# martasumyk/hyperspectral_super-resolution

Hardware: AMD Instinct MI355X
Metric: Mpixel*bands/s fused (SRF + deg-3 per-band LSQ fit + apply) (higher is better)
Workload: dtype f32

## Files before the change

hyperspectral_super-resolution_amd/csrc/hsr_srf.hip:

```cpp
#include <hip/hip_ext.h>

#include "hsr_common.h"
#include "hsr_solve.h"
#include "hsr_sync_dev.h"
#include "hsr_fused_dev.h"

namespace hsr {

struct SrfBands {
  int32_t k0[HSR_MAX_BANDS];
  int32_t klen[HSR_MAX_BANDS];
  int32_t woff[HSR_MAX_BANDS];
  int8_t band_of[8][2];
};

constexpr int kWeightCap = 1024;

typedef hsr_batch_unit SrfUnit;
static_assert(sizeof(SrfUnit) == 64 && sizeof(hsr_batch_tile) == 64, "batch records are 64 bytes");

struct SrfFit {
  double* gpart;
  int32_t* tickets;
  double* moments;
  double* coeffs;
  long long min_count;
};

struct SrfArgs {
  SrfFit fit;
  SrfUnit one;
  const SrfUnit* units;
  int32_t nunits;
  int32_t B;
  int32_t ldsB;
  int32_t wtaps;
  const float* wn;
  SrfBands bands;
  int32_t nb;
  int64_t out_bs, out_ps;
  int64_t real_bs, real_ps;
  float min_x, min_y;
  int32_t u16;
  int32_t u16_fast;
  float scale;
  uint32_t nodata;
  const float* apply_x;
  float* apply_out;
  const double* apply_coeffs;
  const uint8_t* apply_mask;
  int64_t apply_npix;
  int32_t apply_clip;
  const double* lazy_partials;
  int32_t lazy_slots;
  long long lazy_min_count;
  double* lazy_moments;
  double* lazy_coeffs;
  unsigned int* lazy_counter;
  unsigned int lazy_base;
  unsigned int* lazy_ready;
  int32_t lazy_group_T;
  int32_t lazy_group_index;
  const double* lazy_group_moments;
  double* lazy_group_total;
  const unsigned int* apply_ready;
  unsigned int apply_ready_value;
  unsigned int* sync_error;
#ifdef HSR_PHASE_STAMPS
  unsigned long long* stamps;
  unsigned long long* stamps2;
  uint32_t* stamps3;
#endif
};

#ifdef HSR_PHASE_STAMPS
unsigned long long* g_stamp_buffer = nullptr;
unsigned long long* g_stamp_buffer2 = nullptr;
uint32_t* g_stamp_buffer3 = nullptr;
__device__ __forceinline__ unsigned long long real_time() {
  unsigned long long t;
  asm volatile("s_memrealtime %0\n\ts_waitcnt lgkmcnt(0)" : "=s"(t)::"memory");
  return t;
}
__device__ __forceinline__ unsigned long long phase_stamp() {
  unsigned long long t;
  asm volatile("s_memtime %0\n\ts_waitcnt lgkmcnt(0)" : "=s"(t)::"memory");
  return t;
}
#define HSR_STAMP(var) const unsigned long long var = phase_stamp()
#else
#define HSR_STAMP(var)
#endif

constexpr int kGroupPixels = 64;
constexpr int kGroups = 8;
constexpr int kBandSlots = HSR_MAX_BANDS / kGroups;
constexpr int kTapChunk = 16;
constexpr int kScanBatch = 5;
constexpr int kScanBatchF32 = 5;

struct SrfTuning {
  int reserved_cus;
  bool u16_ring;
  bool u16_fast;
};

static int srf_tuning(const hsr_srf_options* o, SrfTuning* t, const char* who) {
  t->reserved_cus = 0;
  t->u16_ring = true;
  t->u16_fast = false;
  if (o == nullptr) return HSR_OK;
  HSR_REQUIRE(o->tile_pixels == 0 || o->tile_pixels == 64, HSR_ERR_INVALID,
              "%s: options.tile_pixels must be 0 (default) or 64, got %d (the 32-pixel geometry of round 1 measured 3-8 %% "
              "slower and was removed)", who, o->tile_pixels);
  HSR_REQUIRE(o->reserved_cus >= 0 && o->reserved_cus <= 128, HSR_ERR_INVALID, "%s: options.reserved_cus=%d outside [0,128]",
              who, o->reserved_cus);
  HSR_REQUIRE((o->flags & ~HSR_SRF_U16_FAST) == 0, HSR_ERR_INVALID, "%s: options.flags has unknown bits (0x%x)", who, o->flags);
  t->reserved_cus = o->reserved_cus;
  t->u16_ring = o->u16_single_buffer == 0;
  t->u16_fast = (o->flags & HSR_SRF_U16_FAST) != 0;
  return HSR_OK;
}

static int srf_slots(int64_t npix, int reserved_cus) {
  int64_t groups = (npix + kGroupPixels - 1) / kGroupPixels;
  if (groups < 1) groups = 1;
  const int64_t cap = (int64_t)(256 - reserved_cus) * 2;
  int64_t slots = groups;
  if (groups > 64 && groups <= 512) {
    slots = (groups + 3) / 4;
    if (slots < 64) slots = 64;
  }
  return (int)(slots < cap ? slots : cap);
}

typedef __attribute__((address_space(1))) const void* gptr_t;
typedef __attribute__((address_space(3))) void* lptr_t;

__device__ __forceinline__ void lds_barrier() {
  asm volatile("s_waitcnt lgkmcnt(0)\n\ts_barrier" ::: "memory");
}

__device__ __forceinline__ void stage_f32(const float* p, float* stage_wave_uniform) {
  __builtin_amdgcn_global_load_lds((gptr_t)p, (lptr_t)stage_wave_uniform, 4, 0, 0);
}
__device__ __forceinline__ void stage_u8(const uint8_t* p, uint32_t* stage_wave_uniform) {
  const uintptr_t a = reinterpret_cast<uintptr_t>(p);
  __builtin_amdgcn_global_load_lds((gptr_t)(a & ~(uintptr_t)3), (lptr_t)stage_wave_uniform, 4, 0, 0);
}
__device__ __forceinline__ uint32_t staged_u8(const uint8_t* p, const uint32_t* stage, int lane) {
  return (stage[lane] >> ((reinterpret_cast<uintptr_t>(p) & 3) * 8)) & 0xffu;
}
constexpr int kTargetStageBytesPerBand = 64 * 4;
__host__ __device__ constexpr size_t target_stage_bytes(int nb) { return (size_t)nb * kTargetStageBytesPerBand + 64 * 4; }

__device__ __forceinline__ const char* unit_record_addr(const SrfUnit* units, int64_t idx, int nunits, int lane) {
  const int64_t i = idx < nunits ? idx : (int64_t)nunits - 1;
  return reinterpret_cast<const char*>(units + i) + (lane & 15) * 4;
}
__device__ __forceinline__ SrfUnit unit_from_lds(const uint32_t* us) {
  uint32_t w[15];
#pragma unroll
  for (int i = 0; i < 15; ++i) w[i] = __builtin_amdgcn_readfirstlane(us[i]);
  SrfUnit u;
  u.cube_dev = reinterpret_cast<const void*>(((uint64_t)w[1] << 32) | w[0]);
  u.real_dev = reinterpret_cast<const float*>(((uint64_t)w[3] << 32) | w[2]);
  u.mask_dev = reinterpret_cast<const uint8_t*>(((uint64_t)w[5] << 32) | w[4]);
  u.pseudo_dev = reinterpret_cast<float*>(((uint64_t)w[7] << 32) | w[6]);
  u.part_dev = reinterpret_cast<double*>(((uint64_t)w[9] << 32) | w[8]);
  u.npix = (int64_t)(((uint64_t)w[11] << 32) | w[10]);
  u.slots = (int32_t)w[12];
  u.slot = (int32_t)w[13];
  u.ngroups = (int32_t)w[14];
  u.reserved = 0;
  return u;
}

__device__ __forceinline__ bool any_nonfinite4(const float4& v) {
  float z = v.x * 0.0f;
  z = fmaf(v.y, 0.0f, z);
  z = fmaf(v.z, 0.0f, z);
  z = fmaf(v.w, 0.0f, z);
  return z != z;
}

__host__ __device__ __forceinline__ int stage_row(int nb, int ops) { return ops > nb ? nb : ops; }

template <int T>
__device__ __forceinline__ void flush_stage(const float* ostage, float* out, int64_t pix0, int npx, int nb, int ops, int t) {
  const int n4 = (npx * ops) >> 2;
  float4* dst = reinterpret_cast<float4*>(out + pix0 * ops);
  if (ops == nb) {
    const float4* src = reinterpret_cast<const float4*>(ostage);
    for (int i = t; i < n4; i += T) st_stream(dst + i, src[i]);
    return;
  }
  const int q = ops >> 2;
  for (int i = t; i < n4; i += T) {
    const int px = q == 4 ? i >> 2 : (q == 2 ? i >> 1 : (q == 1 ? i : i / 3));
    const int c = (i - px * q) * 4;
    const float* r = ostage + px * nb + c;
    st_stream(dst + i, make_float4(c < nb ? r[0] : 0.0f, c + 1 < nb ? r[1] : 0.0f, c + 2 < nb ? r[2] : 0.0f, c + 3 < nb ? r[3] : 0.0f));
  }
}

__device__ __forceinline__ double f64_of(int hi, int lo) { return __hiloint2double(hi, lo); }

template <int D>
__device__ __forceinline__ double merge_pair(double a, double b) {
  const int alo = __double2loint(a), ahi = __double2hiint(a), blo = __double2loint(b), bhi = __double2hiint(b);
  if (D == 32) {
    const auto l = __builtin_amdgcn_permlane32_swap(alo, blo, false, false);
    const auto h = __builtin_amdgcn_permlane32_swap(ahi, bhi, false, false);
    return f64_of(h[0], l[0]) + f64_of(h[1], l[1]);
  } else if (D == 16) {
    const auto l = __builtin_amdgcn_permlane16_swap(alo, blo, false, false);
    const auto h = __builtin_amdgcn_permlane16_swap(ahi, bhi, false, false);
    return f64_of(h[0], l[0]) + f64_of(h[1], l[1]);
  } else if (D == 8) {
    const int xlo = __builtin_amdgcn_update_dpp(alo, blo, 0x128, 0xf, 0xC, false), xhi = __builtin_amdgcn_update_dpp(ahi, bhi, 0x128, 0xf, 0xC, false);
    const int ylo = __builtin_amdgcn_update_dpp(blo, alo, 0x128, 0xf, 0x3, false), yhi = __builtin_amdgcn_update_dpp(bhi, ahi, 0x128, 0xf, 0x3, false);
    return f64_of(xhi, xlo) + f64_of(yhi, ylo);
  } else {
    static_assert(D == 32 || D == 16 || D == 8 || D == 4, "merge levels");
    const int xlo = __builtin_amdgcn_update_dpp(alo, blo, 0x124, 0xf, 0xA, false), xhi = __builtin_amdgcn_update_dpp(ahi, bhi, 0x124, 0xf, 0xA, false);
    const int ylo = __builtin_amdgcn_update_dpp(blo, alo, 0x12C, 0xf, 0x5, false), yhi = __builtin_amdgcn_update_dpp(bhi, ahi, 0x12C, 0xf, 0x5, false);
    return f64_of(xhi, xlo) + f64_of(yhi, ylo);
  }
}

template <int D>
__device__ __forceinline__ double plain_level(double v) {
  const int lo = __double2loint(v), hi = __double2hiint(v);
  if (D == 32) {
    const auto l = __builtin_amdgcn_permlane32_swap(lo, lo, false, false);
    const auto h = __builtin_amdgcn_permlane32_swap(hi, hi, false, false);
    return f64_of(h[0], l[0]) + f64_of(h[1], l[1]);
  }
  static_assert(D == 32 || D == 2 || D == 1, "plain levels");
  constexpr int ctrl = D == 2 ? 0x4E : 0xB1;
  return v + f64_of(__builtin_amdgcn_update_dpp(0, hi, ctrl, 0xf, 0xf, false), __builtin_amdgcn_update_dpp(0, lo, ctrl, 0xf, 0xf, false));
}

template <int D, int NIN, int NMAX>
__device__ __forceinline__ void merge_level(double (&v)[NMAX]) {
  constexpr int NOUT = (NIN + 1) / 2;
#pragma unroll
  for (int i = 0; i < NOUT; ++i) v[i] = merge_pair<D>(v[2 * i], v[2 * i + 1 < NIN ? 2 * i + 1 : NIN - 1]);
}

template <int M, int P, bool LANE_IS_PIXEL, bool COHERENT>
__device__ __forceinline__ void flush_moments(double (&acc_m)[2][M], const bool (&bval)[2], const int (&bidx)[2],
                                              double* part, int lane) {
  constexpr int N = 2 * M;
  constexpr bool kTop32 = P == 64 && LANE_IS_PIXEL;
  constexpr int N1 = kTop32 ? (N + 1) / 2 : N, N2 = (N1 + 1) / 2, N3 = (N2 + 1) / 2, N4 = (N3 + 1) / 2;
  double v[N];
#pragma unroll
  for (int j = 0; j < 2; ++j)
#pragma unroll
    for (int m = 0; m < M; ++m) {
      v[j * M + m] = acc_m[j][m];
      acc_m[j][m] = 0.0;
    }
  if (kTop32) merge_level<32, N, N>(v);
  merge_level<16, N1, N>(v);
  merge_level<8, N2, N>(v);
  merge_level<4, N3, N>(v);
#pragma unroll
  for (int q = 0; q < N4; ++q) {
    v[q] = plain_level<1>(plain_level<2>(v[q]));
    if (!LANE_IS_PIXEL) v[q] = plain_level<32>(v[q]);
  }
  const int b2 = (lane >> 2) & 1, b3 = (lane >> 3) & 1, b4 = (lane >> 4) & 1, b5 = (lane >> 5) & 1;
  const bool canonical = (lane & 3) == 0 && (LANE_IS_PIXEL || b5 == 0);
#pragma unroll
  for (int q = 0; q < N4; ++q) {
    int i = 2 * q + b2;
    bool valid = canonical && i < N3;
    i = 2 * i + b3;
    valid = valid && i < N2;
    i = 2 * i + b4;
    valid = valid && i < N1;
    if (kTop32) {
      i = 2 * i + b5;
      valid = valid && i < N;
    }
    const bool second = i >= M;
    if (valid && (second ? bval[1] : bval[0])) {
      double* dst = part + (size_t)(second ? bidx[1] : bidx[0]) * M + (i - (second ? M : 0));
      if (COHERENT)
        __hip_atomic_store(dst, v[q], __ATOMIC_RELAXED, __HIP_MEMORY_SCOPE_AGENT);
      else
        *dst = v[q];
    }
  }
}

template <int DEG>
__device__ __forceinline__ void fused_fit(const SrfFit& f, const double* part, int S, int nb, unsigned char* lds, int t) {
  constexpr int M = moment_count(DEG);
  const int R = nb * M;
  const int grp = (int)blockIdx.x & 63;
  int* flag = reinterpret_cast<int*>(lds);
  double* mom = reinterpret_cast<double*>(lds + 64);
  double* work = mom + HSR_MAX_BANDS * M;
  stores_done_barrier();
  if (t == 0) {
    const int expect = (S - grp + 63) >> 6;
    *flag = __hip_atomic_fetch_add(f.tickets + grp, 1, __ATOMIC_RELAXED, __HIP_MEMORY_SCOPE_AGENT) == expect - 1;
  }
  __syncthreads();
  if (!*flag) return;
  if (t < R) {
    const double* row = part + t;
    double s = 0.0;
    for (int i0 = grp; i0 < S; i0 += 64 * 8) {
      double v[8];
#pragma unroll
      for (int u = 0; u < 8; ++u) {
        const int i = i0 + 64 * u;
        v[u] = i < S ? ld_agent(row + (size_t)i * R) : 0.0;
      }
#pragma unroll
      for (int u = 0; u < 8; ++u) s += v[u];
    }
    st_agent(f.gpart + (size_t)grp * R + t, s);
  }
  stores_done_barrier();
  const int ngroups = S < 64 ? S : 64;
  if (t == 0) *flag = __hip_atomic_fetch_add(f.tickets + 64, 1, __ATOMIC_RELAXED, __HIP_MEMORY_SCOPE_AGENT) == ngroups - 1;
  __syncthreads();
  if (!*flag) return;
  {
    const int lane = t & 63, wave = t >> 6;
    constexpr int RW = (HSR_MAX_BANDS * M + 7) / 8;
    double v[RW];
#pragma unroll
    for (int k = 0; k < RW; ++k) {
      const int r = wave + 8 * k;
      v[k] = (r < R && lane < ngroups) ? ld_agent(f.gpart + (size_t)lane * R + r) : 0.0;
    }
#pragma unroll
    for (int k = 0; k < RW; ++k) {
      const int r = wave + 8 * k;
      const double s = wave_sum(v[k]);
      if (lane == 0 && r < R) {
        mom[r] = s;
        f.moments[r] = s;
      }
    }
  }
  __syncthreads();
  if (t < nb) solve_band_t<DEG, true>(mom + t * M, f.min_count, f.coeffs + (size_t)t * (DEG + 1), work + t * kSolveWork);
  if (t < 65) __hip_atomic_store(f.tickets + t, 0, __ATOMIC_RELAXED, __HIP_MEMORY_SCOPE_AGENT);
}

template <int DEG, bool FAST, bool WLDS, int P, bool OUTV, bool BATCH, bool APPLY = false>
__global__ __launch_bounds__(8 * P, 4) void srf_kernel(const SrfArgs a) {
  constexpr int T = 8 * P;
  constexpr int NW = T / 64;
  extern __shared__ __attribute__((aligned(16))) unsigned char smem[];
  float* tile = reinterpret_cast<float*>(smem);
  const int B = a.B;
  const int ldsB = a.ldsB;
  uint32_t* flags = reinterpret_cast<uint32_t*>(smem + (size_t)P * ldsB * 4);
  uint32_t* ustage = flags + 64;
  const float* wl = reinterpret_cast<const float*>(flags + 64 + (BATCH ? 16 : 0));
  float* ostage = const_cast<float*>(wl) + (WLDS ? a.wtaps : 0);
  const int ops = (int)a.out_ps;
  const int osr = stage_row(a.nb, ops);
  static_assert(P == 64, "one pixel per lane: the target stage is indexed by lane");
  float* ystage = ostage + (OUTV ? P * osr : 0);
  uint32_t* mstage = reinterpret_cast<uint32_t*>(ystage + a.nb * 64);
  float* prev_out = nullptr;
  int64_t prev_pix0 = 0;
  int prev_npx = 0;

#ifdef HSR_PHASE_STAMPS
  const unsigned long long rt_begin = real_time();
#endif
  const int t = threadIdx.x;
  const int lane = t & 63;
  const int wave = __builtin_amdgcn_readfirstlane(t >> 6);
  const int pl = t % P;
  const int grp = wave;
  const int nchunk = P * B / 4;

  if constexpr (APPLY && DEG > 0) apply_prephase<DEG + 1, T>(a, smem, t);

  int bk0[kBandSlots], bkl[kBandSlots], bwo[kBandSlots], bidx[kBandSlots];
  bool bval[kBandSlots];
#pragma unroll
  for (int j = 0; j < kBandSlots; ++j) {
    const int b = a.bands.band_of[grp][j];
    bval[j] = b >= 0;
    bidx[j] = bval[j] ? b : 0;
    const int bb = bidx[j];
    bk0[j] = a.bands.k0[bb];
    bkl[j] = bval[j] ? a.bands.klen[bb] : 0;
    bwo[j] = a.bands.woff[bb];
  }

  bool constants_staged = false;
  auto stage_constants = [&]() {
    if (WLDS) {
      float* wlw = const_cast<float*>(wl);
      for (int b = 0; b < a.nb; ++b) {
        const int kl = a.bands.klen[b];
        for (int i = t; i < kl; i += T) wlw[a.bands.woff[b] + i] = a.wn[(size_t)b * B + a.bands.k0[b] + i];
      }
    }
  };

#ifdef HSR_PHASE_STAMPS
  unsigned long long stamp_acc[8] = {0, 0, 0, 0, 0, 0, 0, 0};
  unsigned long long round_t0 = rt_begin;
  int round_no = 0;
#endif
  constexpr int M = DEG > 0 ? moment_count(DEG) : 1;
  double acc_m[kBandSlots][M];
  if (DEG > 0) {
#pragma unroll
    for (int j = 0; j < kBandSlots; ++j)
#pragma unroll
      for (int m = 0; m < M; ++m) acc_m[j][m] = 0.0;
  }

  SrfUnit cu;
  if (BATCH) {
    cu = a.units[blockIdx.x];
  } else {
    cu = a.one;
    cu.slot = blockIdx.x;
    cu.part_dev = a.one.part_dev + (size_t)blockIdx.x * a.nb * M;
  }
  int64_t nidx = (int64_t)blockIdx.x + gridDim.x;
  int g = cu.slot;
  bool pend = false;
  double* pend_part = nullptr;

  for (bool more = true; more;) {
    const int64_t pix0 = (int64_t)g * P;
    const int64_t left = cu.npix - pix0;
    const int npx = left < P ? (int)left : P;
    const float* src = reinterpret_cast<const float*>(cu.cube_dev) + pix0 * B;
    const bool pvalid = pl < npx;

    float yv[kBandSlots];
    uint32_t mraw = 1u;
    auto load_targets = [&]() {
      if (DEG > 0) {
        const int64_t pc = pvalid ? pix0 + pl : cu.npix - 1;
#pragma unroll
        for (int j = 0; j < kBandSlots; ++j)
          if (bval[j]) stage_f32(cu.real_dev + bidx[j] * a.real_bs + pc * a.real_ps, ystage + bidx[j] * 64);
        if (cu.mask_dev != nullptr && wave == NW - 1) stage_u8(cu.mask_dev + pc, mstage);
      }
    };
    auto wait_targets = [&]() {
      if (DEG > 0) {
        asm volatile("s_waitcnt vmcnt(0)" ::: "memory");
#pragma unroll
        for (int j = 0; j < kBandSlots; ++j) yv[j] = bval[j] ? ystage[bidx[j] * 64 + lane] : 0.0f;
        mraw = cu.mask_dev != nullptr ? staged_u8(cu.mask_dev + (pvalid ? pix0 + pl : cu.npix - 1), mstage, lane) : 1u;
      }
    };
    auto behind_the_dma = [&]() {
      load_targets();
      if (BATCH && wave == 0 && lane < 16)
        __builtin_amdgcn_global_load_lds((gptr_t)unit_record_addr(a.units, nidx, a.nunits, lane), (lptr_t)ustage, 4, 0, 0);
      if (!constants_staged) {
        stage_constants();
        constants_staged = true;
      }
      if (OUTV) flush_stage<8 * P>(ostage, prev_out, prev_pix0, prev_npx, a.nb, ops, t);
      if (BATCH && DEG > 0 && pend) {
        flush_moments<M, P, true, !BATCH>(acc_m, bval, bidx, pend_part, lane);
        pend = false;
      }
    };

    HSR_STAMP(st0);
    if (t < P) flags[t] = 0u;

    const bool fast_group = FAST && npx == P;
    if (fast_group) {
      const char* srcb = reinterpret_cast<const char*>(src);
      for (int c0 = wave * 64; c0 < nchunk; c0 += T) {
        const int c = c0 + lane;
        if (c < nchunk)
          __builtin_amdgcn_global_load_lds((gptr_t)(srcb + (size_t)c * 16), (lptr_t)(smem + (size_t)c0 * 16),
                                           16, 0, kGldsStream);
      }
    }
    behind_the_dma();
    HSR_STAMP(st1);
    __syncthreads();
    wait_targets();
    HSR_STAMP(st2);
    if (fast_group) {
      const float4* t4 = reinterpret_cast<const float4*>(smem);
      for (int c0 = t; c0 < nchunk; c0 += T * kScanBatchF32) {
        float4 v[kScanBatchF32];
#pragma unroll
        for (int u = 0; u < kScanBatchF32; ++u) {
          const int c = c0 + u * T;
          v[u] = t4[c < nchunk ? c : nchunk - 1];
        }
        bool bad = false;
#pragma unroll
        for (int u = 0; u < kScanBatchF32; ++u) bad |= any_nonfinite4(v[u]);
        if (bad) {
#pragma unroll
          for (int u = 0; u < kScanBatchF32; ++u) {
            const int c = c0 + u * T;
            const int e = (c < nchunk ? c : nchunk - 1) * 4;
            if (!finite_f32(v[u].x)) flags[(e + 0) / B] = 1u;
            if (!finite_f32(v[u].y)) flags[(e + 1) / B] = 1u;
            if (!finite_f32(v[u].z)) flags[(e + 2) / B] = 1u;
            if (!finite_f32(v[u].w)) flags[(e + 3) / B] = 1u;
          }
        }
      }
#ifdef HSR_PHASE_STAMPS
      HSR_STAMP(st3);
      if (a.stamps) { stamp_acc[0] += st1 - st0; stamp_acc[1] += st2 - st1; stamp_acc[2] += st3 - st2; }
#endif
    } else {
      for (int pp = wave; pp < npx; pp += NW) {
        bool bad = false;
        for (int k = lane; k < B; k += 64) {
          const float v = ld_stream(src + (size_t)pp * B + k);
          bad |= !finite_f32(v);
          tile[pp * ldsB + k] = v;
        }
        if (bad) flags[pp] = 1u;
      }
    }
    __syncthreads();

    HSR_STAMP(st4);
    const bool slow = flags[pl] != 0u;
    const float* v = tile + pl * ldsB;
    float accv[kBandSlots];
#pragma unroll
    for (int j = 0; j < kBandSlots; ++j) {
      float acc = 0.0f;
      const float* vs = v + bk0[j];
      if (WLDS) {
        constexpr int CH = kTapChunk / 2;
        const float4* w4 = reinterpret_cast<const float4*>(wl + bwo[j]);
        for (int i0 = 0; i0 < bkl[j]; i0 += CH) {
          float4 ww[CH / 4];
          float xv[CH];
#pragma unroll
          for (int u = 0; u < CH / 4; ++u) ww[u] = w4[(i0 >> 2) + u];
#pragma unroll
          for (int u = 0; u < CH; ++u) xv[u] = vs[i0 + u];
#pragma unroll
          for (int u = 0; u < CH / 4; ++u) {
            acc = fmaf(ww[u].x, xv[4 * u + 0], acc);
            acc = fmaf(ww[u].y, xv[4 * u + 1], acc);
            acc = fmaf(ww[u].z, xv[4 * u + 2], acc);
            acc = fmaf(ww[u].w, xv[4 * u + 3], acc);
          }
        }
      } else {
        const float* ws = a.wn + (size_t)bidx[j] * B + bk0[j];
        for (int i = 0; i < bkl[j]; ++i) acc = fmaf(ws[i], vs[i], acc);
      }
      accv[j] = acc;
    }
    if (slow) {
#pragma unroll
      for (int j = 0; j < kBandSlots; ++j) {
        if (bval[j]) {
          const float* w = a.wn + (size_t)bidx[j] * B;
          float acc = 0.0f;
          for (int k = 0; k < B; ++k) acc = fmaf(w[k], v[k], acc);
          accv[j] = acc;
        }
      }
    }
    if constexpr (!WLDS)
      if (grp == 0 && pvalid && a.out_bs == 1 && ops > a.nb && (ops & 3) == 0 && ops <= HSR_MAX_BANDS &&
          (reinterpret_cast<uintptr_t>(cu.pseudo_dev) & 15) == 0)
        for (int c = a.nb; c < ops; ++c) st_stream(cu.pseudo_dev + (pix0 + pl) * ops + c, 0.0f);
#pragma unroll
    for (int j = 0; j < kBandSlots; ++j) {
      if (bval[j]) {
        const float acc = accv[j];
        if (OUTV) ostage[pl * osr + bidx[j]] = acc;
        else if (pvalid) st_stream(cu.pseudo_dev + bidx[j] * a.out_bs + (pix0 + pl) * a.out_ps, acc);
        if (DEG > 0) {
          const float y = yv[j];
          const bool ok = pvalid && mraw != 0u && finite_f32(acc) && finite_f32(y) && acc > a.min_x && y > a.min_y;
          if (ok) {
            const double xd = (double)acc, yd = (double)y;
            acc_m[j][0] += 1.0;
            acc_m[j][2 * DEG + 1] += yd;
            double pw = 1.0;
#pragma unroll
            for (int k = 1; k <= 2 * DEG; ++k) {
              pw *= xd;
              acc_m[j][k] += pw;
              if (k <= DEG) acc_m[j][2 * DEG + 1 + k] += pw * yd;
            }
          }
        }
      }
    }
    prev_out = cu.pseudo_dev;
    prev_pix0 = pix0;
    prev_npx = npx;
    g += cu.slots;
    if (g >= cu.ngroups) {
      pend = true;
      pend_part = cu.part_dev;
      if (BATCH && nidx < a.nunits) {
        cu = unit_from_lds(ustage);
        g = cu.slot;
        nidx += gridDim.x;
      } else {
        more = false;
      }
    }
    HSR_STAMP(st5);
    lds_barrier();
#ifdef HSR_PHASE_STAMPS
    {
      HSR_STAMP(st6);
      if (a.stamps) { stamp_acc[3] += st5 - st4; stamp_acc[4] += st6 - st5; stamp_acc[5] += st6 - st0; stamp_acc[6] += 1; }
      if (a.stamps3 && t == 0) {
        const unsigned long long now = real_time();
        if (round_no < 64) a.stamps3[(size_t)blockIdx.x * 64 + round_no] = (uint32_t)(now - round_t0);
        round_t0 = now;
        ++round_no;
      }
    }
#endif
  }
  if (OUTV) flush_stage<8 * P>(ostage, prev_out, prev_pix0, prev_npx, a.nb, ops, t);
#ifdef HSR_PHASE_STAMPS
  if (a.stamps && lane == 0)
    for (int k = 0; k < 8; ++k) a.stamps[((size_t)blockIdx.x * NW + wave) * 8 + k] = stamp_acc[k];
#endif
  if (DEG > 0 && pend) flush_moments<M, P, true, !BATCH>(acc_m, bval, bidx, pend_part, lane);
  if constexpr (DEG > 0 && !BATCH)
    if (a.fit.tickets) fused_fit<DEG>(a.fit, a.one.part_dev, a.one.slots, a.nb, smem, t);
  if constexpr (APPLY && DEG > 0)
    if (a.lazy_partials) lazy_fit<DEG, T>(a, smem, t);
#ifdef HSR_PHASE_STAMPS
  if (a.stamps2 && t == 0) {
    uint32_t xcc, hw;
    asm volatile("s_getreg_b32 %0, hwreg(HW_REG_XCC_ID)" : "=s"(xcc));
    asm volatile("s_getreg_b32 %0, hwreg(HW_REG_HW_ID)" : "=s"(hw));
    unsigned long long* o = a.stamps2 + (size_t)blockIdx.x * 4;
    o[0] = rt_begin; o[1] = real_time(); o[2] = xcc; o[3] = hw;
  }
#endif
}


template <int DEG>
__device__ __forceinline__ void moments_accumulate(double (&acc)[DEG > 0 ? moment_count(DEG) : 1], float x, float y) {
  if (DEG == 0) return;
  const double xd = (double)x, yd = (double)y;
  acc[0] += 1.0;
  acc[2 * DEG + 1] += yd;
  double pw = 1.0;
#pragma unroll
  for (int k = 1; k <= 2 * DEG; ++k) {
    pw *= xd;
    acc[k] += pw;
    if (k <= DEG) acc[2 * DEG + 1 + k] += pw * yd;
  }
}

typedef unsigned short u16x2 __attribute__((ext_vector_type(2)));
__device__ __forceinline__ void u16_nodata_sweep(const uint4* t4, int nchunk, int nsamples, int B, uint32_t nd2,
                                                 uint32_t nodata, uint32_t* fl, int t) {
  constexpr int T = 512;
  for (int c0 = t; c0 < nchunk; c0 += T * kScanBatch) {
    uint4 v[kScanBatch];
#pragma unroll
    for (int u = 0; u < kScanBatch; ++u) {
      const int c = c0 + u * T;
      v[u] = t4[c < nchunk ? c : nchunk - 1];
    }
    u16x2 mn = {(unsigned short)0xffffu, (unsigned short)0xffffu};
#pragma unroll
    for (int u = 0; u < kScanBatch; ++u) {
      const uint32_t w[4] = {v[u].x ^ nd2, v[u].y ^ nd2, v[u].z ^ nd2, v[u].w ^ nd2};
#pragma unroll
      for (int q = 0; q < 4; ++q) mn = __builtin_elementwise_min(mn, __builtin_bit_cast(u16x2, w[q]));
    }
    const bool hit = mn.x == 0 || mn.y == 0;
    if (hit) {
#pragma unroll
      for (int u = 0; u < kScanBatch; ++u) {
        const int c = c0 + u * T;
        const int e = (c < nchunk ? c : nchunk - 1) * 8;
        const uint32_t w[4] = {v[u].x, v[u].y, v[u].z, v[u].w};
#pragma unroll
        for (int q = 0; q < 4; ++q) {
          if ((w[q] & 0xffffu) == (nodata & 0xffffu) && e + 2 * q < nsamples) fl[(e + 2 * q) / B] = 1u;
          if ((w[q] >> 16) == (nodata & 0xffffu) && e + 2 * q + 1 < nsamples) fl[(e + 2 * q + 1) / B] = 1u;
        }
      }
    }
  }
}

__device__ __forceinline__ float u16_band_dot(const uint16_t* tile, int e0, const float4* w4, int klen, float scale) {
  float acc = 0.0f;
  const uint32_t sh = (uint32_t)(e0 & 1) * 2u;
  const uint32_t* d32 = reinterpret_cast<const uint32_t*>(tile) + (e0 >> 1);
  for (int i0 = 0; i0 < klen; i0 += kTapChunk) {
    float4 ww[kTapChunk / 4];
    uint32_t d[kTapChunk / 2 + 1];
#pragma unroll
    for (int u = 0; u < kTapChunk / 4; ++u) ww[u] = w4[(i0 >> 2) + u];
#pragma unroll
    for (int u = 0; u <= kTapChunk / 2; ++u) d[u] = d32[(i0 >> 1) + u];
#pragma unroll
    for (int u = 0; u < kTapChunk / 4; ++u) {
      const uint32_t ea = __builtin_amdgcn_alignbyte(d[2 * u + 1], d[2 * u], sh);
      const uint32_t eb = __builtin_amdgcn_alignbyte(d[2 * u + 2], d[2 * u + 1], sh);
      acc = fmaf(ww[u].x, (float)(ea & 0xffffu) * scale, acc);
      acc = fmaf(ww[u].y, (float)(ea >> 16) * scale, acc);
      acc = fmaf(ww[u].z, (float)(eb & 0xffffu) * scale, acc);
      acc = fmaf(ww[u].w, (float)(eb >> 16) * scale, acc);
    }
  }
  return acc;
}

typedef float f32x2 __attribute__((ext_vector_type(2)));
__device__ __forceinline__ float u16_band_dot_fast(const uint16_t* tile, int e0, const float4* w4, int klen) {
  f32x2 acc = {0.0f, 0.0f};
  const uint32_t sh = (uint32_t)(e0 & 1) * 2u;
  const uint32_t* d32 = reinterpret_cast<const uint32_t*>(tile) + (e0 >> 1);
  for (int i0 = 0; i0 < klen; i0 += kTapChunk) {
    float4 ww[kTapChunk / 4];
    uint32_t d[kTapChunk / 2 + 1];
#pragma unroll
    for (int u = 0; u < kTapChunk / 4; ++u) ww[u] = w4[(i0 >> 2) + u];
#pragma unroll
    for (int u = 0; u <= kTapChunk / 2; ++u) d[u] = d32[(i0 >> 1) + u];
#pragma unroll
    for (int u = 0; u < kTapChunk / 4; ++u) {
      const uint32_t ea = __builtin_amdgcn_alignbyte(d[2 * u + 1], d[2 * u], sh);
      const uint32_t eb = __builtin_amdgcn_alignbyte(d[2 * u + 2], d[2 * u + 1], sh);
      const f32x2 x0 = {(float)(ea & 0xffffu), (float)(ea >> 16)}, x1 = {(float)(eb & 0xffffu), (float)(eb >> 16)};
      const f32x2 w0 = {ww[u].x, ww[u].y}, w1 = {ww[u].z, ww[u].w};
      acc = __builtin_elementwise_fma(w0, x0, acc);
      acc = __builtin_elementwise_fma(w1, x1, acc);
    }
  }
  return acc.x + acc.y;
}

template <int DEG, bool FAST, bool OUTV, bool BATCH>
__global__ __launch_bounds__(512, 4) void srf_u16_kernel(const SrfArgs a) {
  constexpr int P = 64, T = 512;
  extern __shared__ __attribute__((aligned(16))) unsigned char smem[];
  uint16_t* tile = reinterpret_cast<uint16_t*>(smem);
  const int B = a.B;
  uint32_t* flags = reinterpret_cast<uint32_t*>(smem + (size_t)P * B * 2);
  uint32_t* ustage = flags + 64;
  const float* wl = reinterpret_cast<const float*>(flags + 64 + (BATCH ? 16 : 0));
  const bool wlds = a.wtaps > 0;
  float* ostage = const_cast<float*>(wl) + a.wtaps;
  const int ops = (int)a.out_ps;
  const int osr = stage_row(a.nb, ops);
  float* ystage = ostage + (OUTV ? P * osr : 0);
  uint32_t* mstage = reinterpret_cast<uint32_t*>(ystage + a.nb * 64);
  float* prev_out = nullptr;
  int64_t prev_pix0 = 0;
  int prev_npx = 0;

  const int t = threadIdx.x;
  const int lane = t & 63;
  const int wave = __builtin_amdgcn_readfirstlane(t >> 6);
  const int pl = 2 * (lane & 31) + (lane >> 5), grp = wave;
  const float scale = a.scale;
  const uint32_t nd2 = (a.nodata & 0xffffu) * 0x00010001u;
  const bool has_nodata = a.nodata <= 0xffffu;

  int bk0[kBandSlots], bkl[kBandSlots], bwo[kBandSlots], bidx[kBandSlots];
  bool bval[kBandSlots];
#pragma unroll
  for (int j = 0; j < kBandSlots; ++j) {
    const int b = a.bands.band_of[grp][j];
    bval[j] = b >= 0;
    bidx[j] = bval[j] ? b : 0;
    bk0[j] = a.bands.k0[bidx[j]];
    bkl[j] = bval[j] ? a.bands.klen[bidx[j]] : 0;
    bwo[j] = a.bands.woff[bidx[j]];
  }
  if (wlds) {
    float* wlw = const_cast<float*>(wl);
    for (int b = 0; b < a.nb; ++b) {
      const int kl = a.bands.klen[b];
      for (int i = t; i < kl; i += T) wlw[a.bands.woff[b] + i] = a.wn[(size_t)b * B + a.bands.k0[b] + i];
    }
  }

  constexpr int M = DEG > 0 ? moment_count(DEG) : 1;
  double acc_m[kBandSlots][M];
  if (DEG > 0) {
#pragma unroll
    for (int j = 0; j < kBandSlots; ++j)
#pragma unroll
      for (int m = 0; m < M; ++m) acc_m[j][m] = 0.0;
  }

  SrfUnit cu;
  if (BATCH) {
    cu = a.units[blockIdx.x];
  } else {
    cu = a.one;
    cu.slot = blockIdx.x;
    cu.part_dev = a.one.part_dev + (size_t)blockIdx.x * a.nb * M;
  }
  int64_t nidx = (int64_t)blockIdx.x + gridDim.x;
  int g = cu.slot;
  bool pend = false;
  double* pend_part = nullptr;

  for (bool more = true; more;) {
    const int64_t pix0 = (int64_t)g * P;
    const int64_t left = cu.npix - pix0;
    const int npx = left < P ? (int)left : P;
    const uint16_t* src = reinterpret_cast<const uint16_t*>(cu.cube_dev) + pix0 * B;
    const bool pvalid = pl < npx;
    const int nchunk = (npx * B + 7) >> 3;

    float yv[kBandSlots];
    uint32_t mraw = 1u;
    auto load_targets = [&]() {
      if (DEG > 0) {
        const int64_t pc = pvalid ? pix0 + pl : cu.npix - 1;
#pragma unroll
        for (int j = 0; j < kBandSlots; ++j)
          if (bval[j]) stage_f32(cu.real_dev + bidx[j] * a.real_bs + pc * a.real_ps, ystage + bidx[j] * 64);
        if (cu.mask_dev != nullptr && wave == 7) stage_u8(cu.mask_dev + pc, mstage);
      }
    };
    auto wait_targets = [&]() {
      if (DEG > 0) {
        asm volatile("s_waitcnt vmcnt(0)" ::: "memory");
#pragma unroll
        for (int j = 0; j < kBandSlots; ++j) yv[j] = bval[j] ? ystage[bidx[j] * 64 + lane] : 0.0f;
        mraw = cu.mask_dev != nullptr ? staged_u8(cu.mask_dev + (pvalid ? pix0 + pl : cu.npix - 1), mstage, lane) : 1u;
      }
    };
    auto behind_the_dma = [&]() {
      load_targets();
      if (BATCH && wave == 0 && lane < 16)
        __builtin_amdgcn_global_load_lds((gptr_t)unit_record_addr(a.units, nidx, a.nunits, lane), (lptr_t)ustage, 4, 0, 0);
      if (OUTV) flush_stage<T>(ostage, prev_out, prev_pix0, prev_npx, a.nb, ops, t);
      if (BATCH && DEG > 0 && pend) {
        flush_moments<M, P, false, !BATCH>(acc_m, bval, bidx, pend_part, lane);
        pend = false;
      }
    };

    if (t < P) flags[t] = 0u;
    const bool fast_group = FAST && npx == P;
    if (fast_group) {
      const char* srcb = reinterpret_cast<const char*>(src);
      for (int c0 = wave * 64; c0 < nchunk; c0 += T) {
        const int c = c0 + lane;
        if (c < nchunk)
          __builtin_amdgcn_global_load_lds((gptr_t)(srcb + (size_t)c * 16), (lptr_t)(smem + (size_t)c0 * 16),
                                           16, 0, kGldsStream);
      }
    }
    behind_the_dma();
    if (!fast_group) {
      const int n = npx * B;
      for (int i = t; i < nchunk * 8; i += T) tile[i] = i < n ? ld_stream(src + i) : (uint16_t)0;
    }
    __syncthreads();
    wait_targets();
    if (has_nodata) {
      u16_nodata_sweep(reinterpret_cast<const uint4*>(smem), nchunk, npx * B, B, nd2, a.nodata, flags, t);
      __syncthreads();
    }

    const bool bad = flags[pl] != 0u;
#pragma unroll
    for (int j = 0; j < kBandSlots; ++j) {
      float acc = 0.0f;
      if (wlds) {
        acc = u16_band_dot(tile, pl * B + bk0[j], reinterpret_cast<const float4*>(wl + bwo[j]), bkl[j], scale);
      } else {
        const uint16_t* vs = tile + pl * B + bk0[j];
        const float* ws = a.wn + (size_t)bidx[j] * B + bk0[j];
        for (int i = 0; i < bkl[j]; ++i) acc = fmaf(ws[i], (float)vs[i] * scale, acc);
      }
      if (bad) acc = __uint_as_float(0x7fc00000u);
      if (bval[j]) {
        if (OUTV) ostage[pl * osr + bidx[j]] = acc;
        else if (pvalid) st_stream(cu.pseudo_dev + bidx[j] * a.out_bs + (pix0 + pl) * a.out_ps, acc);
        if (DEG > 0) {
          const float y = yv[j];
          const bool ok = pvalid && mraw != 0u && finite_f32(acc) && finite_f32(y) && acc > a.min_x && y > a.min_y;
          if (ok) moments_accumulate<DEG>(acc_m[j], acc, y);
        }
      }
    }
    prev_out = cu.pseudo_dev;
    prev_pix0 = pix0;
    prev_npx = npx;
    g += cu.slots;
    if (g >= cu.ngroups) {
      pend = true;
      pend_part = cu.part_dev;
      if (BATCH && nidx < a.nunits) {
        cu = unit_from_lds(ustage);
        g = cu.slot;
        nidx += gridDim.x;
      } else {
        more = false;
      }
    }
    lds_barrier();
  }
  if (OUTV) flush_stage<T>(ostage, prev_out, prev_pix0, prev_npx, a.nb, ops, t);
  if (DEG > 0 && pend) flush_moments<M, P, false, !BATCH>(acc_m, bval, bidx, pend_part, lane);
  if constexpr (DEG > 0 && !BATCH)
    if (a.fit.tickets) fused_fit<DEG>(a.fit, a.one.part_dev, a.one.slots, a.nb, smem, t);
}

__device__ __forceinline__ void glds16_nt_asm(const void* gaddr, uint32_t lds_base) {
  asm volatile("s_mov_b32 m0, %1\n\ts_nop 0\n\tglobal_load_lds_dwordx4 %0, off nt" ::"v"(gaddr), "s"(lds_base) : "memory");
}

__device__ __forceinline__ void glds4_asm(const void* gaddr, uint32_t lds_base) {
  asm volatile("s_mov_b32 m0, %1\n\ts_nop 0\n\tglobal_load_lds_dword %0, off" ::"v"(gaddr), "s"(lds_base) : "memory");
}

constexpr int kU16PrioIssue = 3, kU16PrioDots = 1;
template <int DEG, bool OUTV, bool BATCH, bool FASTU, bool APPLY = false>
__global__ __launch_bounds__(512, 4) void srf_u16_ring_kernel(const SrfArgs a) {
  constexpr int P = 64, T = 512;
  extern __shared__ __attribute__((aligned(16))) unsigned char smem[];
  const int B = a.B;
  const int tile_bytes = P * B * 2;
  uint32_t* flags = reinterpret_cast<uint32_t*>(smem + 2 * (size_t)tile_bytes);
  uint32_t* ustage = flags + 128;
  const float* wl = reinterpret_cast<const float*>(flags + 128 + (BATCH ? 32 : 0));
  const bool wlds = a.wtaps > 0;
  float* ostage = const_cast<float*>(wl) + a.wtaps;
  const int ops = (int)a.out_ps;
  const int osr = stage_row(a.nb, ops);

  const int t = threadIdx.x;
  const int lane = t & 63;
  const int wave = __builtin_amdgcn_readfirstlane(t >> 6);
  const int pl = 2 * (lane & 31) + (lane >> 5), grp = wave;
  const float scale = a.scale;
  const uint32_t nd2 = (a.nodata & 0xffffu) * 0x00010001u;
  const bool has_nodata = a.nodata <= 0xffffu;
  const int nchunk_full = tile_bytes >> 4;

  if constexpr (APPLY && DEG > 0) apply_prephase<DEG + 1, T>(a, smem, t);

  int bk0[kBandSlots], bkl[kBandSlots], bwo[kBandSlots], bidx[kBandSlots];
  bool bval[kBandSlots];
#pragma unroll
  for (int j = 0; j < kBandSlots; ++j) {
    const int b = a.bands.band_of[grp][j];
    bval[j] = b >= 0;
    bidx[j] = bval[j] ? b : 0;
    bk0[j] = a.bands.k0[bidx[j]];
    bkl[j] = bval[j] ? a.bands.klen[bidx[j]] : 0;
    bwo[j] = a.bands.woff[bidx[j]];
  }
  auto stage_constants = [&]() {
    if (wlds) {
      float* wlw = const_cast<float*>(wl);
      for (int b = 0; b < a.nb; ++b) {
        const int kl = a.bands.klen[b];
        for (int i = t; i < kl; i += T) {
          const float wv = a.wn[(size_t)b * B + a.bands.k0[b] + i];
          wlw[a.bands.woff[b] + i] = FASTU ? wv * scale : wv;
        }
      }
    }
  };
  constexpr int M = DEG > 0 ? moment_count(DEG) : 1;
  double acc_m[kBandSlots][M];
  if (DEG > 0) {
#pragma unroll
    for (int j = 0; j < kBandSlots; ++j)
#pragma unroll
      for (int m = 0; m < M; ++m) acc_m[j][m] = 0.0;
  }
  const uint32_t lds0 = (uint32_t)(uintptr_t)(lptr_t)(smem);

  float yn[kBandSlots] = {0.0f, 0.0f};
  uint32_t mn = 1u;
  auto prefetch = [&](const SrfUnit& u, int gg, int buf) {
    const int64_t pix0 = (int64_t)gg * P;
    const int64_t left = u.npix - pix0;
    if (left >= P) {
      const char* srcb = reinterpret_cast<const char*>(reinterpret_cast<const uint16_t*>(u.cube_dev) + pix0 * B);
      for (int c0 = wave * 64; c0 < nchunk_full; c0 += T) {
        const int c = c0 + lane;
        if (c < nchunk_full)
          glds16_nt_asm(srcb + (size_t)c * 16, __builtin_amdgcn_readfirstlane(lds0 + (uint32_t)buf * tile_bytes + (uint32_t)c0 * 16));
      }
    }
    if (DEG > 0) {
      const int64_t pc = pl < left ? pix0 + pl : u.npix - 1;
#pragma unroll
      for (int j = 0; j < kBandSlots; ++j) yn[j] = u.real_dev[bidx[j] * a.real_bs + pc * a.real_ps];
      mn = u.mask_dev != nullptr ? (uint32_t)u.mask_dev[pc] : 1u;
    }
  };

  SrfUnit cu;
  if (BATCH) {
    cu = a.units[blockIdx.x];
  } else {
    cu = a.one;
    cu.slot = blockIdx.x;
    cu.part_dev = a.one.part_dev + (size_t)blockIdx.x * a.nb * M;
  }
  int g = cu.slot;
  prefetch(cu, g, 0);
  stage_constants();
  int64_t nidx = (int64_t)blockIdx.x + gridDim.x;
  auto fetch_record = [&](int64_t idx, int buf) {
    if (BATCH && wave == 0 && lane < 16)
      glds4_asm(unit_record_addr(a.units, idx, a.nunits, lane),
                __builtin_amdgcn_readfirstlane(lds0 + (uint32_t)((const unsigned char*)(ustage + 16 * buf) - smem)));
  };
  fetch_record(nidx, 0);
  int cur = 0;
  float* prev_out = nullptr;
  int64_t prev_pix0 = 0;
  int prev_npx = 0;
  bool pend = false;
  double* pend_part = nullptr;

#ifdef HSR_PHASE_STAMPS
  unsigned long long stamp_acc[8] = {0, 0, 0, 0, 0, 0, 0, 0};
#endif
  for (bool more = true; more; cur ^= 1) {
    HSR_STAMP(st0);
    const int64_t pix0 = (int64_t)g * P;
    const int64_t left = cu.npix - pix0;
    const int npx = left < P ? (int)left : P;
    const bool pvalid = pl < npx;
    const int nchunk = (npx * B + 7) >> 3;
    uint16_t* tile = reinterpret_cast<uint16_t*>(smem + (size_t)cur * tile_bytes);
    uint32_t* fl = flags + 64 * cur;

    if (t < P) fl[t] = 0u;
    asm volatile("s_waitcnt vmcnt(0)" ::: "memory");
    HSR_STAMP(st1);
    float yv[kBandSlots];
    static_assert(kBandSlots == 2, "two target registers");
    yv[0] = yn[0];
    yv[1] = yn[1];
    const uint32_t mraw = mn;
    if (npx < P) {
      const uint16_t* src = reinterpret_cast<const uint16_t*>(cu.cube_dev) + pix0 * B;
      const int n = npx * B;
      for (int i = t; i < nchunk * 8; i += T) tile[i] = i < n ? src[i] : (uint16_t)0;
    }
    __syncthreads();
    HSR_STAMP(st2);

    __builtin_amdgcn_s_setprio(kU16PrioIssue);
    const int g2 = g + cu.slots;
    const bool same_unit = g2 < cu.ngroups;
    const bool next_unit = BATCH && !same_unit && nidx < a.nunits;
    {
      SrfUnit nx = cu;
      int ng = g2;
      if (next_unit) {
        nx = unit_from_lds(ustage + 16 * cur);
        ng = nx.slot;
      }
      if (same_unit || next_unit) prefetch(nx, ng, cur ^ 1);
    }
    fetch_record(next_unit ? nidx + gridDim.x : nidx, cur ^ 1);
    if (OUTV) flush_stage<T>(ostage, prev_out, prev_pix0, prev_npx, a.nb, ops, t);
    if (BATCH && DEG > 0 && pend) {
      flush_moments<M, P, false, !BATCH>(acc_m, bval, bidx, pend_part, lane);
      pend = false;
    }

    HSR_STAMP(st3);
    __builtin_amdgcn_s_setprio(0);
    if (has_nodata) u16_nodata_sweep(reinterpret_cast<const uint4*>(tile), nchunk, npx * B, B, nd2, a.nodata, fl, t);
    lds_barrier();
    HSR_STAMP(st4);

    const bool bad = fl[pl] != 0u;
    __builtin_amdgcn_s_setprio(kU16PrioDots);
#pragma unroll
    for (int j = 0; j < kBandSlots; ++j) {
      float acc = 0.0f;
      if (wlds) {
        acc = FASTU ? u16_band_dot_fast(tile, pl * B + bk0[j], reinterpret_cast<const float4*>(wl + bwo[j]), bkl[j])
                    : u16_band_dot(tile, pl * B + bk0[j], reinterpret_cast<const float4*>(wl + bwo[j]), bkl[j], scale);
      } else {
        const uint16_t* vs = tile + pl * B + bk0[j];
        const float* ws = a.wn + (size_t)bidx[j] * B + bk0[j];
        for (int i = 0; i < bkl[j]; ++i) acc = fmaf(ws[i], (float)vs[i] * scale, acc);
      }
      if (bad) acc = __uint_as_float(0x7fc00000u);
      if (bval[j]) {
        if (OUTV) ostage[pl * osr + bidx[j]] = acc;
        else if (pvalid) st_stream(cu.pseudo_dev + bidx[j] * a.out_bs + (pix0 + pl) * a.out_ps, acc);
        if (DEG > 0) {
          const float y = yv[j];
          const bool ok = pvalid && mraw != 0u && finite_f32(acc) && finite_f32(y) && acc > a.min_x && y > a.min_y;
          if (ok) moments_accumulate<DEG>(acc_m[j], acc, y);
        }
      }
    }
    __builtin_amdgcn_s_setprio(0);
#ifdef HSR_PHASE_STAMPS
    {
      HSR_STAMP(st5);
      if (a.stamps) { stamp_acc[0] += st1 - st0; stamp_acc[1] += st2 - st1; stamp_acc[2] += st3 - st2; stamp_acc[3] += st4 - st3;
                      stamp_acc[4] += st5 - st4; stamp_acc[5] += st5 - st0; stamp_acc[6] += 1; }
    }
#endif
    prev_out = cu.pseudo_dev;
    prev_pix0 = pix0;
    prev_npx = npx;
    if (same_unit) {
      g = g2;
    } else {
      pend = true;
      pend_part = cu.part_dev;
      if (next_unit) {
        cu = unit_from_lds(ustage + 16 * cur);
        g = cu.slot;
        nidx += gridDim.x;
      } else {
        more = false;
      }
    }
  }
#ifdef HSR_PHASE_STAMPS
  if (a.stamps && lane == 0)
    for (int k = 0; k < 8; ++k) a.stamps[((size_t)blockIdx.x * 8 + wave) * 8 + k] = stamp_acc[k];
#endif
  if (OUTV) {
    __syncthreads();
    flush_stage<T>(ostage, prev_out, prev_pix0, prev_npx, a.nb, ops, t);
  }
  if (DEG > 0 && pend) flush_moments<M, P, false, !BATCH>(acc_m, bval, bidx, pend_part, lane);
  if constexpr (DEG > 0 && !BATCH)
    if (a.fit.tickets) fused_fit<DEG>(a.fit, a.one.part_dev, a.one.slots, a.nb, smem, t);
  if constexpr (APPLY && DEG > 0)
    if (a.lazy_partials) lazy_fit<DEG, T>(a, smem, t);
}

typedef void (*SrfKernel)(SrfArgs);
enum SrfVariant {
  kF32Global = 0,
  kF32 = 1,
  kF32Apply = 5,
  kF32Batch = 7,
  kU16 = 9,
  kU16Batch = 13,
  kRing = 15,
  kRingApply = 18,
  kRingBatch = 20,
  kSrfVariants = 22
};
struct SrfKernelRow {
  SrfKernel k[kSrfVariants];
};
template <int D, bool FAST>
constexpr SrfKernel srf_apply_kernel() {
  if constexpr (D > 0) return srf_kernel<D, FAST, true, 64, true, false, true>;
  return nullptr;
}
template <int D, bool FASTU>
constexpr SrfKernel srf_ring_apply_kernel() {
  if constexpr (D > 0) return srf_u16_ring_kernel<D, true, false, FASTU, true>;
  return nullptr;
}
template <int D>
constexpr SrfKernelRow srf_kernel_row() {
  return {{srf_kernel<D, false, false, 64, false, false>,
           srf_kernel<D, false, true, 64, false, false>, srf_kernel<D, false, true, 64, true, false>,
           srf_kernel<D, true, true, 64, false, false>, srf_kernel<D, true, true, 64, true, false>,
           srf_apply_kernel<D, false>(), srf_apply_kernel<D, true>(),
           srf_kernel<D, false, true, 64, true, true>, srf_kernel<D, true, true, 64, true, true>,
           srf_u16_kernel<D, false, false, false>, srf_u16_kernel<D, false, true, false>,
           srf_u16_kernel<D, true, false, false>, srf_u16_kernel<D, true, true, false>,
           srf_u16_kernel<D, false, true, true>, srf_u16_kernel<D, true, true, true>,
           srf_u16_ring_kernel<D, false, false, false>, srf_u16_ring_kernel<D, true, false, false>,
           srf_u16_ring_kernel<D, true, false, true>,
           srf_ring_apply_kernel<D, false>(), srf_ring_apply_kernel<D, true>(),
           srf_u16_ring_kernel<D, true, true, false>, srf_u16_ring_kernel<D, true, true, true>}};
}
static const SrfKernelRow kSrfKernels[HSR_MAX_DEG + 1] = {srf_kernel_row<0>(), srf_kernel_row<1>(), srf_kernel_row<2>(),
                                                          srf_kernel_row<3>(), srf_kernel_row<4>()};
static_assert(HSR_MAX_DEG == 4, "one kernel row per degree");

struct SrfLaunch {
  int deg, variant, grid;
  size_t lds;
  const char* what;
};

static int srf_select(const SrfArgs& a, int deg, const SrfTuning& tn, bool aligned, bool batch, const char* who, SrfLaunch* L) {
  HSR_REQUIRE(deg >= 0 && deg <= HSR_MAX_DEG, HSR_ERR_UNSUPPORTED, "%s: deg=%d outside [0,%d]", who, deg, HSR_MAX_DEG);
  const bool job = !batch && (a.apply_x != nullptr || a.lazy_partials != nullptr);
  HSR_REQUIRE(!job || deg >= 1, HSR_ERR_UNSUPPORTED, "%s: a launch of degree 0 cannot carry an apply job", who);
  HSR_REQUIRE(a.wtaps > 0 || !(job || batch), HSR_ERR_UNSUPPORTED,
              "%s: the weight taps of the %d bands (B=%d) do not fit the %d floats of LDS reserved for them; a batch or a launch "
              "that carries an apply job needs them there", who, a.nb, a.B, kWeightCap);
  const bool outv = batch || (a.out_bs == 1 && (a.out_ps & 3) == 0 && a.out_ps <= HSR_MAX_BANDS && ((uintptr_t)a.one.pseudo_dev & 15) == 0);
  const size_t slab = (size_t)kGroupPixels * stage_row(a.nb, (int)a.out_ps) * 4;
  const size_t weights = (size_t)a.wtaps * 4;
  const size_t single = (64 + (batch ? 16 : 0)) * sizeof(uint32_t) + weights + (deg > 0 ? target_stage_bytes(a.nb) : 0);
  L->deg = deg;
  const int64_t cap = (int64_t)(256 - tn.reserved_cus) * 2;
  L->grid = (int)(a.nunits < cap ? a.nunits : cap);
  if (a.u16) {
    const size_t ring_lds = (size_t)2 * kGroupPixels * a.B * 2 + (128 + (batch ? 32 : 0)) * sizeof(uint32_t) + weights + (outv ? slab : 0);
    const bool ring = aligned && tn.u16_ring && ring_lds <= 80 * 1024;
    HSR_REQUIRE(!job || (ring && outv && 2 * kGroupPixels * a.B * 2 >= 12 * 1024), HSR_ERR_UNSUPPORTED,
                "%s: this launch cannot carry an apply job: uint16 tiles ride only in the double-buffered kernel (16-byte aligned cube, "
                "u16_single_buffer = 0, pixel-major rows, 48 <= B, two %d-byte group buffers + %d taps + the %lld-float rows within "
                "80 KB of LDS)", who, kGroupPixels * a.B * 2, a.wtaps, (long long)a.out_ps);
    const int fastu = a.u16_fast ? 1 : 0;
    if (ring) {
      L->variant = job ? kRingApply + fastu : batch ? kRingBatch + fastu : kRing + (outv ? 1 + (fastu && a.wtaps > 0) : 0);
      L->lds = ring_lds;
      L->what = "srf_u16_ring_kernel launch";
    } else {
      L->variant = batch ? kU16Batch + aligned : kU16 + 2 * aligned + outv;
      L->lds = (size_t)kGroupPixels * a.B * 2 + single + (outv ? slab : 0);
      L->what = "srf_u16_kernel launch";
    }
    return HSR_OK;
  }
  const bool fast = aligned && (a.B & 1);
  const bool staged = a.wtaps > 0 && (outv || job);
  if (a.wtaps == 0) L->variant = kF32Global;
  else if (batch) L->variant = kF32Batch + fast;
  else if (job) L->variant = kF32Apply + fast;
  else L->variant = kF32 + 2 * fast + outv;
  L->lds = (size_t)kGroupPixels * a.ldsB * 4 + single + (staged ? slab : 0);
  L->what = "srf_kernel launch";
  HSR_REQUIRE(!job || L->lds <= 160 * 1024, HSR_ERR_UNSUPPORTED,
              "%s: a 64-pixel group of B=%d samples needs %zu bytes of LDS (160 KB per workgroup)", who, a.B, L->lds);
  return HSR_OK;
}

struct SrfLastLaunch {
  int deg = -1, variant = -1;
  size_t lds = 0;
};
static thread_local SrfLastLaunch g_srf_last;

struct SrfLaunchEvents {
  hipEvent_t start = nullptr, stop = nullptr;
};
static thread_local SrfLaunchEvents g_srf_events;

static int srf_launch(SrfArgs& a, const SrfLaunch& L, hipStream_t stream) {
  const SrfKernel kern = kSrfKernels[L.deg].k[L.variant];
  static thread_local size_t configured[HSR_MAX_DEG + 1][kSrfVariants] = {};
  raise_lds_limit(reinterpret_cast<const void*>(kern), L.lds, configured[L.deg][L.variant]);
#ifdef HSR_PHASE_STAMPS
  a.stamps = g_stamp_buffer;
  a.stamps2 = g_stamp_buffer2;
  a.stamps3 = g_stamp_buffer3;
#endif
  const SrfLaunchEvents ev = g_srf_events;
  g_srf_events = SrfLaunchEvents{};
// ... 456 lines not shown
```

Before: 1.421 million.

## Stage SRF tap weights via async global-to-LDS DMA ahead of apply prephase

Replaces the per-band nested loop that copied SRF weights into LDS through registers with a flat tap-index mapping that issues global_load_lds DMA per tap. In apply+fit variants the copy is issued before the apply prephase so its latency overlaps that work. In the u16 fast path the taps are preloaded into registers early and stored scaled to LDS later. It also adds optional round-0 timing marks under a stamp macro. The costs are extra per-tap band-lookup arithmetic and more register pressure from TapRegs.

```diff
diff --git a/hyperspectral_super-resolution_amd/csrc/hsr_srf.hip b/hyperspectral_super-resolution_amd/csrc/hsr_srf.hip
--- a/hyperspectral_super-resolution_amd/csrc/hsr_srf.hip
+++ b/hyperspectral_super-resolution_amd/csrc/hsr_srf.hip
@@ -88,8 +88,10 @@
   return t;
 }
 #define HSR_STAMP(var) const unsigned long long var = phase_stamp()
+#define HSR_ROUND0_MARK(k) do { if (a.stamps3 && t == 0 && round_no == 0) a.stamps3[(size_t)blockIdx.x * 64 + 48 + (k)] = (uint32_t)(real_time() - rt_begin); } while (0)
 #else
 #define HSR_STAMP(var)
+#define HSR_ROUND0_MARK(k)
 #endif
 
 constexpr int kGroupPixels = 64;
@@ -153,6 +155,56 @@
 }
 constexpr int kTargetStageBytesPerBand = 64 * 4;
 __host__ __device__ constexpr size_t target_stage_bytes(int nb) { return (size_t)nb * kTargetStageBytesPerBand + 64 * 4; }
+
+__device__ __forceinline__ void glds16_nt_asm(const void* gaddr, uint32_t lds_base) {
+  asm volatile("s_mov_b32 m0, %1\n\ts_nop 0\n\tglobal_load_lds_dwordx4 %0, off nt" ::"v"(gaddr), "s"(lds_base) : "memory");
+}
+
+__device__ __forceinline__ void glds4_asm(const void* gaddr, uint32_t lds_base) {
+  asm volatile("s_mov_b32 m0, %1\n\ts_nop 0\n\tglobal_load_lds_dword %0, off" ::"v"(gaddr), "s"(lds_base) : "memory");
+}
+
+__device__ __forceinline__ const float* tap_source(const SrfArgs& a, int c) {
+  int base = 0, end = 0;
+#pragma unroll
+  for (int k = 0; k < HSR_MAX_BANDS; ++k) {
+    const bool in = k < a.nb && c >= a.bands.woff[k];
+    base = in ? k * a.B + a.bands.k0[k] - a.bands.woff[k] : base;
+    end = in ? a.bands.woff[k] + a.bands.klen[k] : end;
+  }
+  return c < end ? a.wn + (base + c) : nullptr;
+}
+enum TapPath { kTapsDma, kTapsDmaAsm };
+template <int T, TapPath PATH>
+__device__ __forceinline__ void stage_taps(const SrfArgs& a, const float* wl, uint32_t wl_lds, int wave, int lane) {
+  for (int c0 = wave * 64; c0 < a.wtaps; c0 += T) {
+    const float* p = tap_source(a, c0 + lane);
+    if (p != nullptr) {
+      if (PATH == kTapsDma) stage_f32(p, const_cast<float*>(wl) + c0);
+      else glds4_asm(p, __builtin_amdgcn_readfirstlane(wl_lds + (uint32_t)c0 * 4));
+    }
+  }
+}
+template <int T>
+struct TapRegs {
+  static constexpr int N = (kWeightCap + T - 1) / T;
+  float v[N];
+  bool ok[N];
+  __device__ __forceinline__ void load(const SrfArgs& a, int t) {
+#pragma unroll
+    for (int u = 0; u < N; ++u) {
+      const int c = t + u * T;
+      const float* p = c < a.wtaps ? tap_source(a, c) : nullptr;
+      ok[u] = p != nullptr;
+      v[u] = ok[u] ? *p : 0.0f;
+    }
+  }
+  __device__ __forceinline__ void store_scaled(const float* wl, int t, float scale) const {
+#pragma unroll
+    for (int u = 0; u < N; ++u)
+      if (ok[u]) const_cast<float*>(wl)[t + u * T] = v[u] * scale;
+  }
+};
 
 __device__ __forceinline__ const char* unit_record_addr(const SrfUnit* units, int64_t idx, int nunits, int lane) {
   const int64_t i = idx < nunits ? idx : (int64_t)nunits - 1;
@@ -387,7 +439,11 @@
   const int grp = wave;
   const int nchunk = P * B / 4;
 
-  if constexpr (APPLY && DEG > 0) apply_prephase<DEG + 1, T>(a, smem, t);
+  constexpr bool kTapsFirst = APPLY && DEG > 0;
+  if constexpr (kTapsFirst) {
+    if (WLDS) stage_taps<T, kTapsDma>(a, wl, 0u, wave, lane);
+    apply_prephase<DEG + 1, T>(a, smem, t);
+  }
 
   int bk0[kBandSlots], bkl[kBandSlots], bwo[kBandSlots], bidx[kBandSlots];
   bool bval[kBandSlots];
@@ -402,15 +458,9 @@
     bwo[j] = a.bands.woff[bb];
   }
 
-  bool constants_staged = false;
+  bool constants_staged = kTapsFirst;
   auto stage_constants = [&]() {
-    if (WLDS) {
-      float* wlw = const_cast<float*>(wl);
-      for (int b = 0; b < a.nb; ++b) {
-        const int kl = a.bands.klen[b];
-        for (int i = t; i < kl; i += T) wlw[a.bands.woff[b] + i] = a.wn[(size_t)b * B + a.bands.k0[b] + i];
-      }
-    }
+    if (WLDS && !kTapsFirst) stage_taps<T, kTapsDma>(a, wl, 0u, wave, lane);
   };
 
 #ifdef HSR_PHASE_STAMPS
@@ -482,6 +532,7 @@
     };
 
     HSR_STAMP(st0);
+    HSR_ROUND0_MARK(0);
     if (t < P) flags[t] = 0u;
 
     const bool fast_group = FAST && npx == P;
@@ -496,9 +547,11 @@
     }
     behind_the_dma();
     HSR_STAMP(st1);
+    HSR_ROUND0_MARK(1);
     __syncthreads();
     wait_targets();
     HSR_STAMP(st2);
+    HSR_ROUND0_MARK(2);
     if (fast_group) {
       const float4* t4 = reinterpret_cast<const float4*>(smem);
       for (int c0 = t; c0 < nchunk; c0 += T * kScanBatchF32) {
@@ -538,6 +591,7 @@
         if (bad) flags[pp] = 1u;
       }
     }
+    HSR_ROUND0_MARK(3);
     __syncthreads();
 
     HSR_STAMP(st4);
@@ -627,6 +681,7 @@
       }
     }
     HSR_STAMP(st5);
+    HSR_ROUND0_MARK(4);
     lds_barrier();
 #ifdef HSR_PHASE_STAMPS
     {
@@ -800,13 +855,7 @@
     bkl[j] = bval[j] ? a.bands.klen[bidx[j]] : 0;
     bwo[j] = a.bands.woff[bidx[j]];
   }
-  if (wlds) {
-    float* wlw = const_cast<float*>(wl);
-    for (int b = 0; b < a.nb; ++b) {
-      const int kl = a.bands.klen[b];
-      for (int i = t; i < kl; i += T) wlw[a.bands.woff[b] + i] = a.wn[(size_t)b * B + a.bands.k0[b] + i];
-    }
-  }
+  stage_taps<T, kTapsDma>(a, wl, 0u, wave, lane);
 
   constexpr int M = DEG > 0 ? moment_count(DEG) : 1;
   double acc_m[kBandSlots][M];
@@ -934,14 +983,6 @@
   if (DEG > 0 && pend) flush_moments<M, P, false, !BATCH>(acc_m, bval, bidx, pend_part, lane);
   if constexpr (DEG > 0 && !BATCH)
     if (a.fit.tickets) fused_fit<DEG>(a.fit, a.one.part_dev, a.one.slots, a.nb, smem, t);
-}
-
-__device__ __forceinline__ void glds16_nt_asm(const void* gaddr, uint32_t lds_base) {
-  asm volatile("s_mov_b32 m0, %1\n\ts_nop 0\n\tglobal_load_lds_dwordx4 %0, off nt" ::"v"(gaddr), "s"(lds_base) : "memory");
-}
-
-__device__ __forceinline__ void glds4_asm(const void* gaddr, uint32_t lds_base) {
-  asm volatile("s_mov_b32 m0, %1\n\ts_nop 0\n\tglobal_load_lds_dword %0, off" ::"v"(gaddr), "s"(lds_base) : "memory");
 }
 
 constexpr int kU16PrioIssue = 3, kU16PrioDots = 1;
@@ -967,8 +1008,22 @@
   const uint32_t nd2 = (a.nodata & 0xffffu) * 0x00010001u;
   const bool has_nodata = a.nodata <= 0xffffu;
   const int nchunk_full = tile_bytes >> 4;
-
-  if constexpr (APPLY && DEG > 0) apply_prephase<DEG + 1, T>(a, smem, t);
+#ifdef HSR_PHASE_STAMPS
+  const unsigned long long rt_begin = real_time();
+#endif
+
+  constexpr bool kTapsFirst = APPLY && DEG > 0;
+  const uint32_t lds0 = (uint32_t)(uintptr_t)(lptr_t)(smem);
+  TapRegs<T> tap_regs;
+  auto stage_constants = [&](bool first) {
+    if (first == kTapsFirst) {
+      if (FASTU) tap_regs.load(a, t);
+      else stage_taps<T, kTapsDmaAsm>(a, wl, lds0 + (uint32_t)((const unsigned char*)wl - smem), wave, lane);
+    }
+    if (FASTU && !first) tap_regs.store_scaled(wl, t, scale);
+  };
+  stage_constants(true);
+  if constexpr (kTapsFirst) apply_prephase<DEG + 1, T>(a, smem, t);
 
   int bk0[kBandSlots], bkl[kBandSlots], bwo[kBandSlots], bidx[kBandSlots];
   bool bval[kBandSlots];
@@ -981,18 +1036,6 @@
     bkl[j] = bval[j] ? a.bands.klen[bidx[j]] : 0;
     bwo[j] = a.bands.woff[bidx[j]];
   }
-  auto stage_constants = [&]() {
-    if (wlds) {
-      float* wlw = const_cast<float*>(wl);
-      for (int b = 0; b < a.nb; ++b) {
-        const int kl = a.bands.klen[b];
-        for (int i = t; i < kl; i += T) {
-          const float wv = a.wn[(size_t)b * B + a.bands.k0[b] + i];
-          wlw[a.bands.woff[b] + i] = FASTU ? wv * scale : wv;
-        }
-      }
-    }
-  };
   constexpr int M = DEG > 0 ? moment_count(DEG) : 1;
   double acc_m[kBandSlots][M];
   if (DEG > 0) {
@@ -1001,8 +1044,6 @@
 #pragma unroll
       for (int m = 0; m < M; ++m) acc_m[j][m] = 0.0;
   }
-  const uint32_t lds0 = (uint32_t)(uintptr_t)(lptr_t)(smem);
-
   float yn[kBandSlots] = {0.0f, 0.0f};
   uint32_t mn = 1u;
   auto prefetch = [&](const SrfUnit& u, int gg, int buf) {
@@ -1034,7 +1075,7 @@
   }
   int g = cu.slot;
   prefetch(cu, g, 0);
-  stage_constants();
+  stage_constants(false);
   int64_t nidx = (int64_t)blockIdx.x + gridDim.x;
   auto fetch_record = [&](int64_t idx, int buf) {
     if (BATCH && wave == 0 && lane < 16)
@@ -1051,6 +1092,8 @@
 
 #ifdef HSR_PHASE_STAMPS
   unsigned long long stamp_acc[8] = {0, 0, 0, 0, 0, 0, 0, 0};
+  unsigned long long round_t0 = rt_begin;
+  int round_no = 0;
 #endif
   for (bool more = true; more; cur ^= 1) {
     HSR_STAMP(st0);
@@ -1134,6 +1177,12 @@
       HSR_STAMP(st5);
       if (a.stamps) { stamp_acc[0] += st1 - st0; stamp_acc[1] += st2 - st1; stamp_acc[2] += st3 - st2; stamp_acc[3] += st4 - st3;
                       stamp_acc[4] += st5 - st4; stamp_acc[5] += st5 - st0; stamp_acc[6] += 1; }
+      if (a.stamps3 && t == 0) {
+        const unsigned long long now = real_time();
+        if (round_no < 64) a.stamps3[(size_t)blockIdx.x * 64 + round_no] = (uint32_t)(now - round_t0);
+        round_t0 = now;
+        ++round_no;
+      }
     }
 #endif
     prev_out = cu.pseudo_dev;
```

New measurement: 1.422 million, median of 2. About the same (+0.0%).
